# DomhnallBoyle/lip2speech-unit

Hardware: AMD Instinct MI355X
Metric: real-time factor (audio-sec/wall-sec), end-to-end lip->16kHz audio, 4s@25fps clips (higher is better)
Workload: dtype fp16; 1 GPU; e2e lip->units->wav (BASELINE configs[3]: AV-HuBERT large 24L + conformer 12x512 + multi_input HiFi-GAN), 4-s 100-frame 88x88 clips, batch 640 per GPU; clips_per_gpu=640, streams=1, clips_per_launch=640, frames_per_clip=100, hipgraph=True, input=uint8 96x96 frames resident in HBM, crop+normalise on device, enc_layers=24, conf_layers=12, parallelism=clip-parallel dp1

## Files before the change

include/lip2speech_hip.h:

```cpp
#ifndef LIP2SPEECH_HIP_H
#define LIP2SPEECH_HIP_H

#include <stddef.h>
#include <stdint.h>

#ifdef __cplusplus
extern "C" {
#endif

#define L2S_ABI_VERSION 16

enum { L2S_F16 = 0, L2S_BF16 = 1, L2S_F32 = 2 };

enum { L2S_OK = 0, L2S_EINVAL = -1, L2S_ESHAPE = -2, L2S_EALIGN = -3, L2S_EUNSUPPORTED = -4 };

enum {
  L2S_ACT_NONE = 0,
  L2S_ACT_RELU = 1,
  L2S_ACT_GELU = 2,
  L2S_ACT_SWISH = 3,
  L2S_ACT_PRELU = 4,
  L2S_ACT_LRELU = 5,
  L2S_ACT_TANH = 6
};
// ... 141 lines not shown
  float slope;
} l2s_respair_final_desc;
int l2s_respair_final(const l2s_respair_final_desc* d, void* stream);

int l2s_basicblock_fused(const void* x, const void* w1, const float* b1, const float* s1, const void* w2, const float* b2,
                         const float* s2, void* y, int n_images, int H, int W, int C, int dtype, void* stream);
int l2s_basiclayer_fused(const void* x, const void* const* w, const float* const* bias, const float* const* slope, int n_blocks,
                         void* y, int n_images, int H, int W, int C, int dtype, void* stream);
int l2s_basicstage128_tail_fused(const void* x0, const void* t0, const void* wa, const float* ba, const float* sa, const void* w1,
                                 const float* b1, const float* s1, const void* w2, const float* b2, const float* s2, void* y,
                                 int n_images, int H, int W, int dtype, void* stream);

int l2s_conv_post_tanh(const float* x, const float* w, float bias, float* wav, int16_t* pcm, const int32_t* lens,
                       int len_mul, int B, int T, int C, int k, void* stream);

int l2s_resblock_fused(const void* xl, const void* w, const float* bias, float* xs, void* xl_out,
                       const int32_t* lens, int len_mul, int B, int T, int C, int k, int d0, int d1, int d2,
                       int accumulate, float slope, int dtype, void* stream);

int l2s_resstage_fused(const void* xl, const void* const* w, const float* const* bias, const int* ks, const int* dils,
                       int n_blocks, float* xs, void* xl_out, const int32_t* lens, int len_mul, int B, int T, int C,
                       float slope, int xs_final, int dtype, void* stream);

int l2s_preprocess_frames(const uint8_t* frames, void* y, int B, int T, int Hin, int Win, int crop, float mean,
                          float std, int dtype, void* stream);

int l2s_mel_spectrogram(const void* wav, int wav_is_i16, int64_t ldw, const int32_t* n_samples, int B, int S, const float* basis,
                        const float* fb, const int32_t* fb_range, float* mel, int ldm, int T_rows, int n_fft, int hop,
                        int n_mels, float floor_, void* stream);

// ... 61 lines not shown
```

lip2speech_unit_amd/_lib.py:

```python
import ctypes
import os

_HERE = os.path.dirname(os.path.abspath(__file__))
LIB_PATH = os.environ.get("L2S_LIB_PATH") or os.path.join(_HERE, "liblip2speech_hip.so")

F16, BF16, F32 = 0, 1, 2
ACT_NONE, ACT_RELU, ACT_GELU, ACT_SWISH, ACT_PRELU, ACT_LRELU, ACT_TANH = range(7)
F_RES_PRE, F_RES_POST, F_ACCUM, F_DUAL, F_MASK, F_OUT_F32, F_RES_F32 = (1 << i for i in range(7))
MODE_LINEAR, MODE_CONV1D, MODE_CONV2D = 0, 1, 2
ABI_VERSION = 16
SEQ_VARIANT_F32, LN_GENERIC, ATTN_RESIDENT = 2000, 10, 1000

_ERR = {-1: "L2S_EINVAL", -2: "L2S_ESHAPE", -3: "L2S_EALIGN", -4: "L2S_EUNSUPPORTED"}


class L2SError(RuntimeError):
    pass


class GemmDesc(ctypes.Structure):
    _fields_ = [
        ("A", ctypes.c_void_p), ("W", ctypes.c_void_p), ("C", ctypes.c_void_p), ("C2", ctypes.c_void_p),
        ("bias", ctypes.c_void_p), ("slope", ctypes.c_void_p), ("R", ctypes.c_void_p), ("lens", ctypes.c_void_p),
        ("M", ctypes.c_int32), ("N", ctypes.c_int32), ("Cin", ctypes.c_int32), ("ntaps", ctypes.c_int32),
# ... 60 lines not shown
    "l2s_splitk_reduce": ([_vp, _i, _i, _vp, _i, _i, _i, _vp], _i),
    "l2s_splitk_reduce_layernorm": ([_vp, _i, _i, _vp, _i, _vp, _vp, _f, _vp, _i, _i, _i, _i, _vp, _i, _i, _i, _vp], _i),
    "l2s_cast_f32_to_16": ([_vp, _i, _vp, _i, _i, _i, _i, _vp], _i),
    "l2s_cast_16_to_f32": ([_vp, _i, _vp, _i, _i, _i, _i, _vp], _i),
    "l2s_broadcast_rows": ([_vp, _i, _vp, _i, _i, _vp, _i, _i, _i, _i, _i, _i, _vp], _i),
    "l2s_transpose_ct_to_tc": ([_vp, _vp, _i, _i, _vp, _i, _i, _i, _i, _i, _vp], _i),
    "l2s_embedding": ([_vp, _vp, _vp, _i, _vp, _i, _i, _i, _i, _vp], _i),
    "l2s_embedding_tokens": ([_vp, _i, _i, _vp, _i, _vp, _i, _vp, _i, _i, _i, _i, _i, _vp], _i),
    "l2s_rows_f32_to_16_masked": ([_vp, _i, _vp, _i, _i, _vp, _i, _i, _i, _i, _i, _vp], _i),
    "l2s_lens_from_mask": ([_vp, _vp, _i, _i, _vp], _i),
    "l2s_basicblock_fused": ([_vp, _vp, _vp, _vp, _vp, _vp, _vp, _vp, _i, _i, _i, _i, _i, _vp], _i),
    "l2s_basiclayer_fused": ([_vp, _vp, _vp, _vp, _i, _vp, _i, _i, _i, _i, _i, _vp], _i),
    "l2s_basicstage128_tail_fused": ([_vp] * 12 + [_i, _i, _i, _i, _vp], _i),
    "l2s_split_hi_lo": ([_vp, _i, _vp, _vp, _i, _i, _f, _vp, _i, _i, _i, _i, _i, _vp], _i),
    "l2s_conv_post_tanh": ([_vp, _vp, _f, _vp, _vp, _vp, _i, _i, _i, _i, _i, _vp], _i),
    "l2s_resblock_fused": ([_vp, _vp, _vp, _vp, _vp, _vp, _i, _i, _i, _i, _i, _i, _i, _i, _i, _f, _i, _vp], _i),
    "l2s_resstage_fused": ([_vp, _vp, _vp, _vp, _vp, _i, _vp, _vp, _vp, _i, _i, _i, _i, _f, _i, _i, _vp], _i),
    "l2s_respair": ([ctypes.POINTER(RespairDesc), _vp], _i),
    "l2s_respair_variant": ([ctypes.POINTER(RespairDesc)], _i),
    "l2s_respair_final": ([ctypes.POINTER(RespairFinalDesc), _vp], _i),
    "l2s_preprocess_frames": ([_vp, _vp, _i, _i, _i, _i, _i, _f, _f, _i, _vp], _i),
    "l2s_mel_spectrogram": ([_vp, _i, ctypes.c_int64, _vp, _i, _i, _vp, _vp, _vp, _vp, _i, _i, _i, _i, _i, _f, _vp], _i),
    "l2s_stft_mel": ([_vp, _i, ctypes.c_int64, _vp, _i, _i, _vp, _vp, _vp, _vp, _i, _i, _i, _i, _i, _i, _f, _f, _vp], _i),
    "l2s_unit_ce": ([_vp, _i, _vp, _i, _vp, _i, _i, _i, _i, _i, _i, _vp, _vp, _vp, _vp, _vp], _i),
    "l2s_mel_l1_sc": ([_vp, _i, _vp, _i, _vp, _i, _i, _i, _i, _vp, _vp, _vp, _vp, _vp], _i),
    "l2s_ctc_loss_workspace": ([_i, _i, _i], ctypes.c_size_t),
    "l2s_ctc_loss": ([_vp, _i, _vp, _i, _i, _i, _i, _i, _vp, _vp, _vp, _i, _vp, ctypes.c_size_t, _vp, _vp], _i),
    "l2s_wave_stem_workspace": ([_i, _i], ctypes.c_size_t),
    "l2s_wave_stem": ([_vp, _i, ctypes.c_int64, _vp, _i, _i, _vp, _vp, _vp, _f, _vp, _i, _i, _i, _vp, ctypes.c_size_t, _i, _vp], _i),
    "l2s_kmeans_assign": ([_vp, _i, _vp, _vp, _vp, _i, _i, _i, _i, _i, _vp, _vp, _vp], _i),
# ... 51 lines not shown
```

lip2speech_unit_amd/ops.py:

```python
import ctypes
import os
from typing import Optional

import torch

from . import _lib
from ._lib import (ACT_GELU, ACT_LRELU, ACT_NONE, ACT_PRELU, ACT_RELU, ACT_SWISH, ACT_TANH, BF16, F16, F32, F_ACCUM,
                   F_DUAL, F_MASK, F_OUT_F32, F_RES_F32, F_RES_POST, F_RES_PRE, MODE_CONV1D, MODE_CONV2D,
                   MODE_LINEAR, GemmDesc, L2SError, check)

_TORCH16 = {F16: torch.float16, BF16: torch.bfloat16, F32: torch.float32}
_DTYPE_NAME = {F16: "f16", BF16: "bf16", F32: "f32"}


class KernelProfiler:

    def __init__(self, detail=False):
        self.records = []
        self.detail = detail

    def summary(self):
        torch.cuda.synchronize()
        agg = {}
        for key, fl, by, e0, e1, shape in self.records:
# ... 375 lines not shown
    sp = (ctypes.c_void_p * n)(*[_ptr(_req(s_, torch.float32, "slope")) for s_ in slopes])
    M = float(n_images) * H * W
    _run("l2s_basiclayer_fused", lambda: _lib.load().l2s_basiclayer_fused(
        _ptr(x), wp, bp, sp, n // 2, _ptr(y), n_images, H, W, C, dtype, _stream()),
        flops=2.0 * n * M * C * C * 9, nbytes=2 * 2 * M * C)


def split_hi_lo(x, hi, lo, *, B, T, C, act=0, slope=0.0, ldx=None, ld16=None, lens=None, len_mul=1, dtype=F16):
    _run("l2s_split_hi_lo", lambda: _lib.load().l2s_split_hi_lo(_ptr(x), ldx or C, _ptr(hi), _ptr(lo), ld16 or C, act, float(slope),
                                                                _ptr(lens), len_mul, B, T, C, dtype, _stream()))


def conv_post_tanh(x, w, bias, wav, pcm, *, B, T, C, k, lens=None, len_mul=1):
    _run("l2s_conv_post_tanh", lambda: _lib.load().l2s_conv_post_tanh(_ptr(x), _ptr(w), float(bias), _ptr(wav), _ptr(pcm), _ptr(lens), len_mul, B,
                                         T, C, k, _stream()))


def resblock_fused(xl, w, bias, xs, xl_out, *, B, T, C, k, dil, accumulate, slope, lens=None, len_mul=1, dtype=F16):
    _run(f"l2s_resblock_fused<C{C},k{k}>", lambda: _lib.load().l2s_resblock_fused(
        _ptr(xl), _ptr(w), _ptr(bias), _ptr(xs), _ptr(xl_out), _ptr(lens), len_mul, B, T, C, k, dil[0], dil[1], dil[2],
        int(bool(accumulate)), float(slope), dtype, _stream()),
        flops=2.0 * B * T * C * C * k * 6, nbytes=B * T * C * (2 + 4 + (4 if accumulate else 0) + (2 if xl_out is not None else 0)))


def resstage_fused(xl, ws, biases, xs, xl_out, *, B, T, C, ks, dils, slope, lens=None, len_mul=1, dtype=F16, xs_final=True):
    n = len(ws)
    wp = (ctypes.c_void_p * n)(*[_ptr(_req(w, _TORCH16[dtype], "w")) for w in ws])
    bp = (ctypes.c_void_p * n)(*[_ptr(_req(b_, torch.float32, "bias")) for b_ in biases])
    kk = (ctypes.c_int * n)(*[int(k) for k in ks])
    dd = (ctypes.c_int * (3 * n))(*[int(d) for dl in dils for d in dl])
# ... 538 lines not shown
    "embedding_tokens": "(Tensor tok, Tensor table, Tensor(a!) y, *, int B, int L, int C, int token_offset=4, int? ldt=None, "
                        "int? ldy=None, Tensor? lens=None, int len_mul=1, int dtype=0) -> ()",
    "rows_f32_to_16_masked": "(Tensor x, Tensor(a!) y, *, int B, int T, int C, int? ldx=None, int? ldy=None, int col0=0, "
                             "Tensor? lens=None, int len_mul=1, int dtype=0) -> ()",
    "lens_from_mask": "(Tensor? padding_mask, int B, int T, Device device) -> Tensor",
    "basicblock_fused": "(Tensor x, Tensor w1, Tensor b1, Tensor s1, Tensor w2, Tensor b2, Tensor s2, Tensor(a!) y, *, int n_images, "
                        "int H, int W, int C=64, int dtype=0) -> ()",
    "basiclayer_fused": _BL,
    "basicstage128_tail_fused": "(Tensor x0, Tensor t0, Tensor wa, Tensor ba, Tensor sa, Tensor w1, Tensor b1, Tensor s1, Tensor w2, "
                                "Tensor b2, Tensor s2, Tensor(a!) y, *, int n_images, int H, int W, int dtype=0) -> ()",
    "split_hi_lo": "(Tensor x, Tensor(a!) hi, Tensor(b!) lo, *, int B, int T, int C, int act=0, float slope=0.0, int? ldx=None, "
                   "int? ld16=None, Tensor? lens=None, int len_mul=1, int dtype=0) -> ()",
    "conv_post_tanh": _CPT,
    "resblock_fused": "(Tensor xl, Tensor w, Tensor bias, Tensor(a!) xs, Tensor(b!)? xl_out, *, int B, int T, int C, int k, int[] dil, "
                      "bool accumulate, float slope, Tensor? lens=None, int len_mul=1, int dtype=0) -> ()",
    "resstage_fused": "(Tensor xl, Tensor[] ws, Tensor[] biases, Tensor(a!) xs, Tensor(b!)? xl_out, *, int B, int T, int C, int[] ks, "
                      "int[] dils, float slope, Tensor? lens=None, int len_mul=1, int dtype=0, bool xs_final=True) -> ()",
    "respair": _RP,
    "respair_final": "(Tensor[] xs_l, Tensor[] w1s, Tensor[] b1s, Tensor[] w2s, Tensor[] b2s, Tensor(a!) y, *, int B, int T, int C, int[] ks, "
                     "int[] dils, float slope, Tensor? lens=None, int len_mul=1, int dtype=0) -> ()",
    "preprocess_frames": "(Tensor frames, Tensor(a!) y, *, int B, int T, int Hin, int Win, int crop=88, float mean=0.421, "
                         "float std=0.165, int dtype=0) -> ()",
    "mel_spectrogram": "(Tensor wav, Tensor(a!) mel, Tensor basis, Tensor fb, Tensor fb_range, *, int B, int S, int T_rows, "
                       "Tensor? n_samples=None, int? ldw=None, int? ldm=None, int n_fft=640, int hop=160, int n_mels=80, "
                       "float floor=1e-05) -> ()",
    "stft_mel": "(Tensor wav, Tensor(a!) mel, Tensor basis, Tensor fb, Tensor fb_range, *, int B, int S, int T_rows, int n_fft, int hop, "
                "int pad, float mag_eps=0.0, Tensor? n_samples=None, int? ldw=None, int? ldm=None, int n_mels=80, "
                "float floor=1e-05) -> ()",
    "unit_ce": "(Tensor logits, Tensor target, Tensor(a!) nll, Tensor(b!) smooth, Tensor(c!) n_correct, Tensor(d!) n_tok, *, int B, "
               "int T2, int V, int? ldl=None, int? ldt=None, Tensor? lens=None, int len_mul=2, int pad_idx=1, "
# ... 22 lines not shown
                  "int B, int S, int ldf, Tensor? n_samples=None, int? ldx=None, int? ldk=None) -> ()",
    "stoi_scores": "(Tensor bands, Tensor n_kept, Tensor(a!) seg, Tensor(b!) stoi, Tensor(c!) estoi, Tensor(d!) n_segments, *, int B, "
                   "int ldf, int? lds=None) -> ()",
    "wav_gain": "(Tensor wav, Tensor(a!) gain, *, int B, int S, Tensor? n_samples=None, int? ldw=None, float target_dbfs=-30.0) -> ()",
    "stft_mel_power": "(Tensor wav, Tensor(a!) mel, Tensor basis, Tensor fb, Tensor fb_range, *, int B, int S, int T_rows, "
                      "Tensor? n_samples=None, Tensor? n_valid=None, Tensor? scale=None, int? ldw=None, int? ldm=None, int n_fft=400, "
                      "int hop=160, int n_mels=40, int pad=200) -> ()",
    "lstm_layer": "(Tensor xproj, Tensor row_off, Tensor w_hh_p, *, int S, int T, int? n_rows=None, int? ldx=None, int hidden=256, "
                  "Tensor(a!)? h_seq=None, Tensor(b!)? h_last=None) -> ()",
    "spk_embed_head": "(Tensor h_last, Tensor first, Tensor count, Tensor w_t, Tensor bias, Tensor(a!) out, *, int B, "
                      "int? n_rows=None, int hidden=256) -> ()",
}
ENTRY_OF = {n: "l2s_" + n for n in _SCHEMAS}
ENTRY_OF.update({"maxpool2d_3x3s2": "l2s_maxpool2d_3x3s2", "avgpool_hw": "l2s_avgpool_hw"})
HOST_QUERIES = ("l2s_abi_version", "l2s_build_info", "l2s_tapgemm_variant", "l2s_tapgemm_epilogue_family", "l2s_attention_variant", "l2s_layernorm_variant", "l2s_respair_variant",
                "l2s_glu_dwconv_tile", "l2s_beam_decode_workspace",
                "l2s_ctc_beam_workspace", "l2s_ctc_loss_workspace", "l2s_wave_stem_workspace", "l2s_kmeans_nearest_workspace",
                "l2s_kmeans_update_workspace", "l2s_kmeans_pp_workspace")
ALIASES = {"frontend3d_stem": "stem_pool_fused", "resnet_trunk": "basiclayer_fused", "linear_epilogue": "tapgemm",
           "posconv_gelu": "tapgemm", "convtranspose1d": "tapgemm", "mel_head": "tapgemm", "mhsa_padmask": "attention",
           "relpos_mhsa": "attention", "conformer_conv_module": "glu_dwconv_swish", "greedy_unit_decode": "greedy_decode",
           "resblock1": "respair", "tanh_to_int16": "conv_post_tanh"}

_TORCH_LIB = torch.library.Library("lip2speech", "DEF")


def _fake_none(*a, **k):
    return None


def _fake_beam_decode(logits, *, B, T2, V, beam, ldl=None, lens=None, len_mul=1, temperature=1.0, lenpen=1.0):
# ... 58 lines not shown
```

lip2speech_unit_amd/packing.py:

```python
import itertools
from typing import Dict, List

import torch

_clock = itertools.count(1)


def _device(dev):
    dev = torch.device(dev)
    if dev.type == "cuda" and dev.index is None:
        dev = torch.device("cuda", torch.cuda.current_device())
    return dev


def _invalidate_on_load(module, incompatible_keys):
    module.invalidate()


class PackedState:

    def _init_packed(self):
        self._packed, self._packed_dev, self._derived = None, None, {}
        self._epoch = next(_clock)
        self.register_load_state_dict_post_hook(_invalidate_on_load)
# ... 61 lines not shown
        for j in range(p["ntaps"]):
            i = d_max - (p["off"] - j)
            wf[p["r"] * cout:(p["r"] + 1) * cout, i] = wp[:, j]
    if fold == 1:
        return {"w": wf.reshape(stride * cout, S * cin).contiguous(), "ntaps": S, "off": d_max, "n": stride * cout, "fold": 1}
    f, N = fold, stride * cout
    D_max, D_min = (f - 1 + d_max) // f, (d_max - (S - 1)) // f
    S2 = D_max - D_min + 1
    w2 = torch.zeros(f * N, S2, f * cin, dtype=w.dtype)
    for b in range(f):
        for i in range(S):
            m = b + d_max - i
            D, a = m // f, m % f
            w2[b * N:(b + 1) * N, D_max - D, a * cin:(a + 1) * cin] = wf[:, i]
    return {"w": w2.reshape(f * N, S2 * f * cin).contiguous(), "ntaps": S2, "off": D_max, "n": f * N, "fold": f}
```

lip2speech_unit_amd/vocoder.py:

```python
import os

import torch
import torch.nn as nn

from . import ops
from .ops import ACT_GELU, ACT_LRELU, F_ACCUM, F_DUAL, F_MASK, F_RES_POST, MODE_CONV1D
from .packing import PackedState, convtranspose_fused, convtranspose_phases, pack_conv1d

LRELU_SLOPE = 0.1
FUSED_PAIR = os.environ.get("L2S_RESPAIR", "1") != "0"
FUSED_PAIR256 = os.environ.get("L2S_RESPAIR256", "1") != "0"
PAIR_MIN_TILES = int(os.environ.get("L2S_RESPAIR_MIN_TILES", "64"))
PAIR_ROWS = {256: 128, 128: 256, 64: 512}
FUSED_UPS = os.environ.get("L2S_FUSED_UPS", "1") != "0"
FUSED_UPS_MAX_CIN = int(os.environ.get("L2S_FUSED_UPS_MAX_CIN", "128"))
FUSED_STAGE = os.environ.get("L2S_RESSTAGE", "1") != "0"
FUSED_FINAL = os.environ.get("L2S_RESPAIR_FINAL", "1") != "0"
SKIP_DEAD_XS = os.environ.get("L2S_SKIP_DEAD_XS", "1") != "0"


class AttrDict(dict):

    def __init__(self, *args, **kwargs):
        super().__init__(*args, **kwargs)
        self.__dict__ = self


def get_padding(kernel_size, dilation=1):
    return int((kernel_size * dilation - dilation) / 2)

# ... 5 lines not shown
        self.weight_g = nn.Parameter(torch.ones(g_dim0, 1, 1))
        self.weight_v = nn.Parameter(torch.zeros(*shape))
        self.bias = nn.Parameter(torch.zeros(bias_n))

    def effective_weight(self):
        if hasattr(self, "weight") and isinstance(getattr(self, "weight"), torch.Tensor):
            return self.weight.detach().float()
        v, g = self.weight_v.detach().float(), self.weight_g.detach().float()
        return v * (g / v.pow(2).sum(dim=(1, 2), keepdim=True).sqrt())

    def remove_weight_norm(self):
        if "weight_g" in self._parameters:
            w = self.effective_weight()
            del self._parameters["weight_g"], self._parameters["weight_v"]
            self.weight = nn.Parameter(w)


class ResBlock1(nn.Module):
    def __init__(self, h, channels, kernel_size=3, dilation=(1, 3, 5)):
        super().__init__()
        self.channels, self.kernel_size, self.dilation = channels, kernel_size, tuple(dilation)
        self.convs1 = nn.ModuleList([_WN((channels, channels, kernel_size), channels, channels) for _ in dilation])
        self.convs2 = nn.ModuleList([_WN((channels, channels, kernel_size), channels, channels) for _ in dilation])

    def remove_weight_norm(self):
        for m in list(self.convs1) + list(self.convs2):
            m.remove_weight_norm()


class Generator(nn.Module, PackedState):
# ... 25 lines not shown
        for m in self.ups:
            m.remove_weight_norm()
        for m in self.resblocks:
            m.remove_weight_norm()
        self.conv_pre.remove_weight_norm()
        self.conv_post.remove_weight_norm()
        self.invalidate()

    def _conv_pre_weight(self):
        return self.conv_pre.effective_weight()

    def _pack_generator(self, dev):
        t16 = ops.torch_dtype(self.dtype)
        h = self.h
        third = 1.0 / self.num_kernels
        P = {"pre_w": pack_conv1d(self._conv_pre_weight()).to(dev, t16).contiguous(),
             "pre_b": self.conv_pre.bias.detach().float().to(dev).contiguous(), "stages": []}
        for i, (u, k) in enumerate(zip(h.upsample_rates, h.upsample_kernel_sizes)):
            w = self.ups[i].effective_weight()
            if i > 0:
                w = w * third
            st = {"u": u, "cout": w.shape[1], "cin": w.shape[0],
                  "phases": [dict(ph, w=ph["w"].to(dev, t16).contiguous()) for ph in
                             convtranspose_phases(w, u, (k - u) // 2)],
                  "b": self.ups[i].bias.detach().float().to(dev).contiguous(), "rbs": []}
            if FUSED_UPS and w.shape[0] <= FUSED_UPS_MAX_CIN:
                fold = 2 if (w.shape[0] == 32 and u * w.shape[1] == 32) else 1
                f = convtranspose_fused(w, u, (k - u) // 2, fold=fold)
                st["fused"] = dict(f, w=f["w"].to(dev, t16).contiguous(), b=st["b"].repeat(u * fold).contiguous())
            for j in range(self.num_kernels):
                rb = self.resblocks[i * self.num_kernels + j]
                convs = []
                for c1, c2, d in zip(rb.convs1, rb.convs2, rb.dilation):
                    convs.append({
                        "w1": pack_conv1d(c1.effective_weight()).to(dev, t16).contiguous(),
                        "b1": c1.bias.detach().float().to(dev).contiguous(), "d": d,
                        "w2": pack_conv1d(c2.effective_weight()).to(dev, t16).contiguous(),
                        "b2": c2.bias.detach().float().to(dev).contiguous()})
                e = {"k": rb.kernel_size, "convs": convs, "dil": tuple(rb.dilation)}
                C = w.shape[1]
                if C in (16, 32) and rb.kernel_size in (3, 7, 11) and len(rb.dilation) == 3:
                    kpad = ((rb.kernel_size * C + 31) // 32) * 32
                    wf = torch.zeros(6, C, kpad)
                    bf = torch.zeros(6, C)
# ... 82 lines not shown
        P, dt = self._packed["gen"], self.dtype
        t16 = ops.torch_dtype(dt)
        dev = x_l.device
        T, mul = T0, base_mul
        xs = None
        for si, st in enumerate(P["stages"]):
            u, C = st["u"], st["cout"]
            To, M_in = T * u, B * T
            mul *= u
            M = B * To
            pair_stage = FUSED_PAIR and (C in (64, 128) or (C == 256 and FUSED_PAIR256)) and all(
                rb["k"] <= 11 and max(rb["dil"]) * (rb["k"] - 1) // 2 <= (28 if C == 256 else 32) for rb in st["rbs"])
            pair_stage = pair_stage and B * -(-To // PAIR_ROWS[C]) >= PAIR_MIN_TILES
            fused_stage = all("fw" in rb for rb in st["rbs"])
            xl = torch.empty(M, C, device=dev, dtype=t16)
            if (pair_stage or fused_stage) and "fused" in st:
                x, f = None, st["fused"]
                fd = f["fold"] if T % f["fold"] == 0 and (mul // u) % f["fold"] == 0 else 0
                if fd == 0:
                    raise ops.L2SError("folded ConvTranspose needs an even number of input steps per clip")
                ops.tapgemm(x_l, f["w"], xl, M=M_in // fd, N=f["n"], Cin=st["cin"] * fd, ntaps=f["ntaps"], mode=MODE_CONV1D,
                            T_out=T // fd, T_in=T // fd, stride=1, dil=-1, off=f["off"], bias=f["b"], act=ACT_LRELU,
                            act_slope=LRELU_SLOPE, lens=lens, mask_T=T // fd, mask_mul=mul // u // fd, flags=F_MASK, dtype=dt)
            elif pair_stage or fused_stage:
                x = None
                for ph in st["phases"]:
                    ops.tapgemm(x_l, ph["w"], xl, M=M_in, N=C, Cin=st["cin"], ntaps=ph["ntaps"], mode=MODE_CONV1D, T_out=T,
                                T_in=T, stride=1, dil=-1, off=ph["off"], out_row_mul=u, out_row_add=ph["r"], bias=st["b"],
                                act=ACT_LRELU, act_slope=LRELU_SLOPE, lens=lens, mask_T=To, mask_mul=mul, flags=F_MASK,
                                dtype=dt)
            else:
                x = torch.empty(M, C, device=dev, dtype=t16)
                for ph in st["phases"]:
                    ops.tapgemm(x_l, ph["w"], x, M=M_in, N=C, Cin=st["cin"], ntaps=ph["ntaps"], mode=MODE_CONV1D, T_out=T,
                                T_in=T, stride=1, dil=-1, off=ph["off"], out_row_mul=u, out_row_add=ph["r"], bias=st["b"],
                                C2=xl, ldc2=C, lens=lens, mask_T=To, mask_mul=mul, flags=F_DUAL | F_MASK,
                                slope2=LRELU_SLOPE, dtype=dt)
            nxt = torch.empty(M, C, device=dev, dtype=t16)
            last_stage = si == len(P["stages"]) - 1
            final_fused = pair_stage and FUSED_FINAL and SKIP_DEAD_XS and not last_stage and len(st["rbs"]) <= 3
            xs = None if final_fused else torch.empty(M, C, device=dev, dtype=torch.float32)
            if pair_stage:
                finals = []
                for j, rb in enumerate(st["rbs"]):
                    cur_l = xl
# ... 148 lines not shown
        fw = torch.zeros(Etp, Etp)
        fw[:Et, :Et] = fc.weight.detach().float().cpu()
        fb = torch.zeros(Etp)
        fb[:Et] = fc.bias.detach().float().cpu()
        return table, cw, cb, fw, fb

    def pack(self, dev):
        t16 = ops.torch_dtype(self.dtype)
        P = {"gen": self._pack_generator(dev)}
        P["table"] = self.dict.weight.detach().to(dev, t16).contiguous()
        ct = self.layer[0]
        P["up_phases"] = [dict(ph, w=ph["w"].to(dev, t16).contiguous())
                          for ph in convtranspose_phases(ct.weight.detach().float(), 2, 1)]
        P["up_b"] = ct.bias.detach().float().to(dev).contiguous()
        P["fc_w"], P["fc_b"] = self.fc.weight.detach().to(dev, t16).contiguous(), self.fc.bias.detach().float().to(dev).contiguous()
        P["sp_w"], P["sp_b"] = self.spkr.weight.detach().to(dev, t16).contiguous(), self.spkr.bias.detach().float().to(dev).contiguous()
        if self.text_supervision:
            table, cw, cb, fw, fb = self._text_weights()
            P["t_table"] = table.to(dev, t16).contiguous()
            P["t_phases"] = [dict(ph, w=ph["w"].to(dev, t16).contiguous()) for ph in convtranspose_phases(cw, 2, 1)]
            P["t_up_b"], P["t_fc_w"], P["t_fc_b"] = cb.to(dev), fw.to(dev, t16).contiguous(), fb.to(dev)
        self._set_packed(dev, P)

    def _check_text(self, t):
        if self.text_supervision and t is None:
            raise ValueError("this vocoder is text-supervised (models_multi_input.py:75-77): pass the frame labels (t_label)")
        if t is not None and not self.text_supervision:
            raise ValueError("frame labels given to a vocoder without text supervision")

    def forward_rows(self, code, mel, spkr, lens=None, t_label=None):
        dev = code.device
# ... 82 lines not shown
            assert t_rows.dtype == torch.int32 and t_rows.shape[0] == B and t_rows.shape[1] >= L and t_rows.stride(1) == 1
            text = (t_rows, t_rows.stride(0), src_lens, 2)

        def fill(P, cat, emb, Cin, dt):
            ops.embedding_tokens(tokens, P["table"], emb, B=B, L=L, C=self.h.embedding_dim, token_offset=token_offset,
                                 ldt=tokens.stride(0), lens=src_lens, len_mul=2, dtype=dt)
            ops.rows_f32_to_16_masked(mel_rows, cat, B=B, T=2 * L, C=nm, ldy=Cin, col0=0, lens=src_lens, len_mul=4, dtype=dt)
        return self._rows(fill, spkr, src_lens, 2, B, L, dev, text)

    def _rows(self, fill, spkr, lens, lm, B, L, dev, text=None):
        P, dt, h = self.packed(dev), self.dtype, self.h
        t16 = ops.torch_dtype(dt)
        E, nm = h.embedding_dim, self.num_mels
        T0 = 2 * L
        Ct = P["t_table"].shape[1] if self.text_supervision else 0
        Cin = nm + 2 * E + Ct
        cat = torch.empty(B * T0, Cin, device=dev, dtype=t16)
        emb = torch.empty(B * L, E, device=dev, dtype=t16)
        fill(P, cat, emb, Cin, dt)
        up = torch.empty(B * T0, E, device=dev, dtype=t16)
        for ph in P["up_phases"]:
            ops.tapgemm(emb, ph["w"], up, M=B * L, N=E, Cin=E, ntaps=ph["ntaps"], mode=MODE_CONV1D, T_out=L, T_in=L,
                        stride=1, dil=-1, off=ph["off"], out_row_mul=2, out_row_add=ph["r"], bias=P["up_b"],
                        act=ACT_GELU, lens=lens, mask_T=T0, mask_mul=2 * lm, flags=F_MASK, dtype=dt)
        ops.tapgemm(up, P["fc_w"], cat[:, nm:], M=B * T0, N=E, Cin=E, ldc=Cin, bias=P["fc_b"], lens=lens, mask_T=T0,
                    mask_mul=2 * lm, flags=F_MASK, dtype=dt)
        if Ct:
            tok, ldt, tlens, tmul = text
            temb = torch.empty(B * L, Ct, device=dev, dtype=t16)
            ops.embedding_tokens(tok, P["t_table"], temb, B=B, L=L, C=Ct, token_offset=0, ldt=ldt, lens=tlens, len_mul=tmul,
                                 dtype=dt)
            tup = torch.empty(B * T0, Ct, device=dev, dtype=t16)
            for ph in P["t_phases"]:
                ops.tapgemm(temb, ph["w"], tup, M=B * L, N=Ct, Cin=Ct, ntaps=ph["ntaps"], mode=MODE_CONV1D, T_out=L, T_in=L,
                            stride=1, dil=-1, off=ph["off"], out_row_mul=2, out_row_add=ph["r"], bias=P["t_up_b"],
                            act=ACT_GELU, lens=lens, mask_T=T0, mask_mul=2 * lm, flags=F_MASK, dtype=dt)
            ops.tapgemm(tup, P["t_fc_w"], cat[:, nm + E:], M=B * T0, N=Ct, Cin=Ct, ldc=Cin, bias=P["t_fc_b"], lens=lens,
                        mask_T=T0, mask_mul=2 * lm, flags=F_MASK, dtype=dt)
        spkr = spkr.contiguous()
        if spkr.dtype == torch.float32:
            sp16 = torch.empty(B, spkr.shape[1], device=dev, dtype=t16)
            ops.cast_f32_to_16(spkr, sp16, B, spkr.shape[1], dt)
        else:
            sp16 = spkr.to(t16)
        sp = torch.empty(B, E, device=dev, dtype=t16)
        ops.tapgemm(sp16, P["sp_w"], sp, M=B, N=E, Cin=sp16.shape[1], bias=P["sp_b"], dtype=dt)
        ops.broadcast_rows(sp, cat, B=B, T=T0, C=E, ldy=Cin, col0=nm + E + Ct, lens=lens, len_mul=2 * lm, dtype=dt)
        G = P["gen"]
        c0 = G["pre_b"].shape[0]
        x_l = torch.empty(B * T0, c0, device=dev, dtype=t16)
        ops.tapgemm(cat, G["pre_w"], x_l, M=B * T0, N=c0, Cin=Cin, ntaps=7, mode=MODE_CONV1D, T_out=T0, T_in=T0,
                    stride=1, dil=1, off=-3, bias=G["pre_b"], act=ACT_LRELU, act_slope=LRELU_SLOPE, lens=lens,
                    mask_T=T0, mask_mul=2 * lm, flags=F_MASK, dtype=dt)
        return self.generator_rows(x_l, lens, B, T0, 2 * lm)

    def forward(self, **kwargs):
        wav, _ = self.forward_rows(kwargs["code"], kwargs["mel"], kwargs["spkr"], kwargs.get("lens"), t_label=kwargs.get("t_label"))
        return wav.unsqueeze(1)
```

Before: 14080 audio-sec/wall-sec.

## Add dedicated upsample+LReLU kernel with k-step sparsity masks and pad conv_pre Cin

Measured after the change: 14150 audio-sec/wall-sec (median of 6 runs). No clear change (+0.5%).

```diff
diff --git a/include/lip2speech_hip.h b/include/lip2speech_hip.h
--- a/include/lip2speech_hip.h
+++ b/include/lip2speech_hip.h
@@ -179,6 +179,10 @@
 int l2s_conv_post_tanh(const float* x, const float* w, float bias, float* wav, int16_t* pcm, const int32_t* lens,
                        int len_mul, int B, int T, int C, int k, void* stream);
 
+int l2s_upsample_lrelu(const void* x, const void* w, const float* bias, void* y, const int32_t* lens, int len_mul, int B, int T,
+                       int Cin, int N, int ntaps, int off, const uint32_t* kmask, float slope, int dtype, void* stream);
+int l2s_upsample_tile(int Cin, int N);
+
 int l2s_resblock_fused(const void* xl, const void* w, const float* bias, float* xs, void* xl_out,
                        const int32_t* lens, int len_mul, int B, int T, int C, int k, int d0, int d1, int d2,
                        int accumulate, float slope, int dtype, void* stream);
diff --git a/lip2speech_unit_amd/_lib.py b/lip2speech_unit_amd/_lib.py
--- a/lip2speech_unit_amd/_lib.py
+++ b/lip2speech_unit_amd/_lib.py
@@ -98,6 +98,8 @@
     "l2s_basicstage128_tail_fused": ([_vp] * 12 + [_i, _i, _i, _i, _vp], _i),
     "l2s_split_hi_lo": ([_vp, _i, _vp, _vp, _i, _i, _f, _vp, _i, _i, _i, _i, _i, _vp], _i),
     "l2s_conv_post_tanh": ([_vp, _vp, _f, _vp, _vp, _vp, _i, _i, _i, _i, _i, _vp], _i),
+    "l2s_upsample_lrelu": ([_vp, _vp, _vp, _vp, _vp, _i, _i, _i, _i, _i, _i, _i, _vp, _f, _i, _vp], _i),
+    "l2s_upsample_tile": ([_i, _i], _i),
     "l2s_resblock_fused": ([_vp, _vp, _vp, _vp, _vp, _vp, _i, _i, _i, _i, _i, _i, _i, _i, _i, _f, _i, _vp], _i),
     "l2s_resstage_fused": ([_vp, _vp, _vp, _vp, _vp, _i, _vp, _vp, _vp, _i, _i, _i, _i, _f, _i, _i, _vp], _i),
     "l2s_respair": ([ctypes.POINTER(RespairDesc), _vp], _i),
diff --git a/lip2speech_unit_amd/csrc/upsample.hip b/lip2speech_unit_amd/csrc/upsample.hip
--- /dev/null
+++ b/lip2speech_unit_amd/csrc/upsample.hip
@@ -0,0 +1,277 @@
+#include "tapgemm_common.h"
+#include <cstdlib>
+
+using namespace l2s;
+
+namespace {
+
+struct UpsArgs {
+  const uint16_t* X; const uint16_t* W; const float* bias; uint16_t* Y; const int32_t* lens;
+  int len_mul, B, T, tile_rows, tiles_per_clip, ntiles;
+  float slope;
+};
+
+constexpr int UPS_TAPS = 3;
+
+template <int CIN, int N>
+struct UpsCfg {
+  static constexpr int WC = (CIN == 128) ? 4 : 1;
+  static constexpr int WM = 4 / WC;
+  static constexpr int NP = N / 32 / WC;
+  static constexpr int MI = (CIN == 128) ? 8 : 4;
+  static constexpr int TM = WM * MI * 16;
+  static constexpr int PROWS = TM + 8;
+  static constexpr int HALVES = CIN / 64;
+  static constexpr int PLANE_B = PROWS * 128;
+  static constexpr int BUF_B = HALVES * PLANE_B;
+  static constexpr int SMEM = 2 * BUF_B;
+  static constexpr int KS = UPS_TAPS * CIN / 32;
+};
+
+template <typename ET, int CIN, int N, uint64_t MASKS, int NT, unsigned TBS>
+__global__ __launch_bounds__(256, 2) void upsample_lrelu_kernel(const UpsArgs a) {
+  using C = UpsCfg<CIN, N>;
+  constexpr int MI = C::MI, NP = C::NP, KPT = CIN / 32, KS = NT * KPT, K = UPS_TAPS * CIN;
+  static_assert(C::WC == 1 || NP == 1, "a wave's pairs share one tap window");
+  extern __shared__ __attribute__((aligned(16))) uint16_t lds[];
+  const int tid = threadIdx.x, lane = tid & 63;
+  const int wave = __builtin_amdgcn_readfirstlane(tid >> 6);
+  const int lm = lane & 15, lg = lane >> 4;
+  const int srow = lane >> 3, schunk = (lane & 7) ^ (srow & 7);
+  const int wm = wave / C::WC, wc = wave - wm * C::WC;
+  const uint16_t* zero = reinterpret_cast<const uint16_t*>(&g_zero16);
+  const int my_n = (a.ntiles - (int)blockIdx.x + (int)gridDim.x - 1) / (int)gridDim.x;
+  if (my_n <= 0) return;
+  const uint32_t lds_base = (uint32_t)(uintptr_t)(lptr_t)lds;
+
+  auto pair_mask = [](int jp) -> unsigned { return (unsigned)((MASKS >> (12 * jp)) & 0xfffu); };
+  const int tb = (int)((TBS >> (2 * (wc * NP))) & 3u);
+  auto tile_origin = [&](int i, int& b, int& q0) {
+    const int L = blockIdx.x + i * gridDim.x;
+    b = __builtin_amdgcn_readfirstlane(L / a.tiles_per_clip);
+    q0 = (L - b * a.tiles_per_clip) * a.tile_rows;
+  };
+  auto issue_patch = [&](int i, int buf) {
+    int b, q0;
+    tile_origin(i, b, q0);
+    constexpr int NINS = C::HALVES * (C::PROWS / 8);
+    for (int ins = wave; ins < NINS; ins += 4) {
+      const int hp = ins / (C::PROWS / 8), blk = ins - hp * (C::PROWS / 8);
+      const int ts = q0 - 1 + blk * 8 + srow;
+      const uint16_t* g = ((unsigned)ts < (unsigned)a.T) ? a.X + ((int64_t)b * a.T + ts) * CIN + hp * 64 + schunk * 8 : zero;
+      __builtin_amdgcn_global_load_lds((gptr_t)g, (lptr_t)(lds + (buf * C::BUF_B + hp * C::PLANE_B + blk * 1024) / 2), 16, 0, 0);
+    }
+  };
+
+  frag16 wf[NP][2][KS];
+  f32x4_t bj[NP][2];
+#pragma unroll
+  for (int jp = 0; jp < NP; ++jp) {
+    const int J = wc * NP + jp;
+#pragma unroll
+    for (int s2 = 0; s2 < 2; ++s2) {
+      const int n = 32 * J + 8 * (lm >> 2) + 4 * s2 + (lm & 3);
+#pragma unroll
+      for (int s = 0; s < KS; ++s)
+        if ((pair_mask(jp) >> s) & 1u) wf[jp][s2][s].u = *reinterpret_cast<const uint4*>(a.W + (int64_t)n * K + tb * CIN + s * 32 + lg * 8);
+      const float4 q = *reinterpret_cast<const float4*>(a.bias + 32 * J + 8 * lg + 4 * s2);
+      bj[jp][s2] = f32x4_t{q.x, q.y, q.z, q.w};
+    }
+  }
+#pragma unroll
+  for (int jp = 0; jp < NP; ++jp)
+#pragma unroll
+    for (int s2 = 0; s2 < 2; ++s2) {
+#pragma unroll
+      for (int s = 0; s < KS; ++s)
+        if ((pair_mask(jp) >> s) & 1u) asm volatile("" : "+v"(wf[jp][s2][s].h));
+      asm volatile("" : "+v"(bj[jp][s2]));
+    }
+  uint32_t aoff[KS];
+#pragma unroll
+  for (int s = 0; s < KS; ++s) {
+    const int tl = s / KPT, kk = s - tl * KPT, hp = kk >> 1, ks2 = kk & 1;
+    const int pr = wm * MI * 16 + lm + 2 - (tb + tl);
+    aoff[s] = (uint32_t)(hp * C::PLANE_B + pr * 128 + (((ks2 * 4 + lg) ^ (pr & 7)) << 4));
+  }
+  constexpr unsigned ANY = [] {
+    unsigned m = 0;
+    for (int jp = 0; jp < NP; ++jp) m |= (unsigned)((MASKS >> (12 * jp)) & 0xfffu);
+    return m;
+  }();
+
+  issue_patch(0, 0);
+  f32x4_t acc[MI][2 * NP];
+  frag16 fa[2][MI];
+  auto read_a = [&](int s, int slot, uint32_t pb) {
+    const uint32_t ad = pb + aoff[s];
+    lds_read_b128<0>(fa[slot][0], ad); lds_read_b128<2048>(fa[slot][1], ad);
+    lds_read_b128<4096>(fa[slot][2], ad); lds_read_b128<6144>(fa[slot][3], ad);
+    if constexpr (MI == 8) {
+      lds_read_b128<8192>(fa[slot][4], ad); lds_read_b128<10240>(fa[slot][5], ad);
+      lds_read_b128<12288>(fa[slot][6], ad); lds_read_b128<14336>(fa[slot][7], ad);
+    }
+  };
+
+  for (int it = 0; it < my_n; ++it) {
+    wait_vmcnt<0>();
+    __builtin_amdgcn_s_barrier();
+    asm volatile("" ::: "memory");
+    if (it + 1 < my_n) issue_patch(it + 1, (it + 1) & 1);
+    const uint32_t pb = lds_base + (uint32_t)((it & 1) * C::BUF_B);
+#pragma unroll
+    for (int i = 0; i < MI; ++i)
+#pragma unroll
+      for (int j = 0; j < 2 * NP; ++j) acc[i][j] = f32x4_t{0.f, 0.f, 0.f, 0.f};
+
+    constexpr int FIRST = __builtin_ctz(ANY);
+    read_a(FIRST, 0, pb);
+    int slot = 0;
+#pragma unroll
+    for (int s = 0; s < KS; ++s) {
+      if (!((ANY >> s) & 1u)) continue;
+      int nxt = -1;
+#pragma unroll
+      for (int s3 = KS - 1; s3 > s; --s3)
+        if ((ANY >> s3) & 1u) nxt = s3;
+      if (nxt >= 0) {
+        read_a(nxt, slot ^ 1, pb);
+        lds_wait_n<MI>();
+      } else {
+        lds_wait_n<0>();
+      }
+#pragma unroll
+      for (int jp = 0; jp < NP; ++jp) {
+        if ((pair_mask(jp) >> s) & 1u) {
+#pragma unroll
+          for (int i = 0; i < MI; ++i) {
+            acc[i][2 * jp] = ET::mfma(wf[jp][0][s], fa[slot][i], acc[i][2 * jp]);
+            acc[i][2 * jp + 1] = ET::mfma(wf[jp][1][s], fa[slot][i], acc[i][2 * jp + 1]);
+          }
+        }
+      }
+      slot ^= 1;
+    }
+
+    int b, q0;
+    tile_origin(it, b, q0);
+    int valid = a.T;
+    if (a.lens) {
+      int len_b;
+      const int32_t* lp = a.lens + b;
+      asm volatile("s_load_dword %0, %1, 0x0\n\ts_waitcnt lgkmcnt(0)" : "=s"(len_b) : "s"(lp) : "memory");
+      const int v = len_b * a.len_mul;
+      valid = v < a.T ? v : a.T;
+    }
+    const int row_end = (q0 + a.tile_rows < a.T) ? q0 + a.tile_rows : a.T;
+    uint16_t* yrow = a.Y + ((int64_t)b * a.T + q0) * N + wc * NP * 32 + 8 * lg;
+    const float slope = a.slope;
+#pragma unroll
+    for (int i = 0; i < MI; ++i) {
+      const int g0 = q0 + (wm * MI + i) * 16;
+      if (g0 >= row_end) break;
+      const int q = g0 + lm;
+      const bool st = q < row_end;
+      uint16_t* dst = yrow + (int64_t)((wm * MI + i) * 16 + lm) * N;
+      if (g0 >= valid) {
+        if (st) {
+#pragma unroll
+          for (int jp = 0; jp < NP; ++jp) *reinterpret_cast<uint4*>(dst + 32 * jp) = make_uint4(0u, 0u, 0u, 0u);
+        }
+        continue;
+      }
+      const bool partial = g0 + 16 > valid;
+#pragma unroll
+      for (int jp = 0; jp < NP; ++jp) {
+        float v[8];
+#pragma unroll
+        for (int e = 0; e < 8; ++e) {
+          const float x = acc[i][2 * jp + (e >> 2)][e & 3] + bj[jp][e >> 2][e & 3];
+          v[e] = __builtin_amdgcn_fmed3f(x, x * slope, __builtin_inff());
+        }
+        uint4 pk = make_uint4(ET::pack2(v[0], v[1]), ET::pack2(v[2], v[3]), ET::pack2(v[4], v[5]), ET::pack2(v[6], v[7]));
+        if (partial && q >= valid) pk = make_uint4(0u, 0u, 0u, 0u);
+        if (st) *reinterpret_cast<uint4*>(dst + 32 * jp) = pk;
+      }
+    }
+  }
+  wait_vmcnt<0>();
+}
+
+constexpr uint64_t mask4(unsigned m0, unsigned m1, unsigned m2, unsigned m3) {
+  return (uint64_t)m0 | ((uint64_t)m1 << 12) | ((uint64_t)m2 << 24) | ((uint64_t)m3 << 36);
+}
+constexpr uint64_t M64_PHASES = mask4(0x3c, 0x0f, 0, 0);
+constexpr uint64_t M64_FOLD2 = mask4(0x2c, 0x0d, 0, 0);
+constexpr uint64_t M64_DENSE = mask4(0x3f, 0x3f, 0, 0);
+constexpr unsigned TB128_PHASES = 1u | (1u << 2);
+
+bool covers(uint64_t masks, int nt, unsigned tbs, int kpt, int np_wave, const uint32_t* kmask, int npairs) {
+  if (!kmask) return false;
+  for (int J = 0; J < npairs; ++J) {
+    const unsigned local = (unsigned)((masks >> (12 * (J % np_wave))) & 0xfffu) & ((1u << (nt * kpt)) - 1u);
+    const unsigned global = local << (((tbs >> (2 * J)) & 3u) * kpt);
+    if (kmask[J] & ~global) return false;
+  }
+  return true;
+}
+
+int ups_tile_rows(int Cin, int N) {
+  int tm = 0;
+  if (Cin == 64 && N == 64) tm = UpsCfg<64, 64>::TM;
+  if (Cin == 128 && N == 128) tm = UpsCfg<128, 128>::TM;
+  if (!tm) return 0;
+  const char* e = getenv("L2S_UPS_TILE");
+  const int v = e ? atoi(e) : 0;
+  return (v >= 16 && v < tm && v % 16 == 0) ? v : tm;
+}
+
+template <typename ET, int CIN, int N, uint64_t MASKS, int NT, unsigned TBS>
+int launch_ups(UpsArgs a, hipStream_t st) {
+  using C = UpsCfg<CIN, N>;
+  auto kern = upsample_lrelu_kernel<ET, CIN, N, MASKS, NT, TBS>;
+  static L2sSmemOptIn opt_in;
+  if (int e = l2s_smem_opt_in(kern, C::SMEM, opt_in)) return e;
+  constexpr int resident = 512;
+  const char* e = getenv("L2S_UPS_SLOTS");
+  const int sv = e ? atoi(e) : 0;
+  const int slots = sv >= 1 && sv < resident ? sv : resident;
+  const int grid = a.ntiles < slots ? a.ntiles : slots;
+  hipLaunchKernelGGL(kern, dim3(grid), dim3(256), C::SMEM, st, a);
+  L2S_CHECK_LAUNCH();
+  return L2S_OK;
+}
+
+template <typename ET>
+int launch_ups_shape(const UpsArgs& a, int Cin, const uint32_t* kmask, hipStream_t st) {
+  if (Cin == 64) {
+    if (covers(M64_FOLD2, 3, 0, 2, 2, kmask, 2)) return launch_ups<ET, 64, 64, M64_FOLD2, 3, 0>(a, st);
+    if (covers(M64_PHASES, 3, 0, 2, 2, kmask, 2)) return launch_ups<ET, 64, 64, M64_PHASES, 3, 0>(a, st);
+    return launch_ups<ET, 64, 64, M64_DENSE, 3, 0>(a, st);
+  }
+  if (covers(0xff, 2, TB128_PHASES, 4, 1, kmask, 4)) return launch_ups<ET, 128, 128, 0xff, 2, TB128_PHASES>(a, st);
+  return launch_ups<ET, 128, 128, 0xfff, 3, 0>(a, st);
+}
+
+}
+extern "C" int l2s_upsample_tile(int Cin, int N) { return ups_tile_rows(Cin, N); }
+
+extern "C" int l2s_upsample_lrelu(const void* x, const void* w, const float* bias, void* y, const int32_t* lens, int len_mul, int B,
+                                  int T, int Cin, int N, int ntaps, int off, const uint32_t* kmask, float slope, int dtype,
+                                  void* stream) {
+  if (!x || !w || !bias || !y) return L2S_EINVAL;
+  if (B <= 0 || T <= 0 || len_mul <= 0) return L2S_ESHAPE;
+  if (dtype != L2S_F16 && dtype != L2S_BF16) return dtype == L2S_F32 ? L2S_EUNSUPPORTED : L2S_EINVAL;
+  const int tile = ups_tile_rows(Cin, N);
+  if (!tile || ntaps != UPS_TAPS || off != 1 || !(slope > 0.f && slope <= 1.f)) return L2S_EUNSUPPORTED;
+  if ((int64_t)B * T > 0x7fffffff / 2) return L2S_EUNSUPPORTED;
+  if ((((uintptr_t)x | (uintptr_t)w | (uintptr_t)y | (uintptr_t)bias) & 15) != 0) return L2S_EALIGN;
+  UpsArgs a;
+  a.X = (const uint16_t*)x; a.W = (const uint16_t*)w; a.bias = bias; a.Y = (uint16_t*)y; a.lens = lens;
+  a.len_mul = len_mul; a.B = B; a.T = T; a.tile_rows = tile;
+  a.tiles_per_clip = (T + tile - 1) / tile;
+  a.ntiles = B * a.tiles_per_clip;
+  a.slope = slope;
+  hipStream_t st = (hipStream_t)stream;
+  return dtype == L2S_F16 ? launch_ups_shape<ElemF16>(a, Cin, kmask, st) : launch_ups_shape<ElemBF16>(a, Cin, kmask, st);
+}
diff --git a/lip2speech_unit_amd/ops.py b/lip2speech_unit_amd/ops.py
--- a/lip2speech_unit_amd/ops.py
+++ b/lip2speech_unit_amd/ops.py
@@ -413,6 +413,27 @@
 def conv_post_tanh(x, w, bias, wav, pcm, *, B, T, C, k, lens=None, len_mul=1):
     _run("l2s_conv_post_tanh", lambda: _lib.load().l2s_conv_post_tanh(_ptr(x), _ptr(w), float(bias), _ptr(wav), _ptr(pcm), _ptr(lens), len_mul, B,
                                          T, C, k, _stream()))
+
+
+def upsample_tile(Cin, N):
+    return _lib.load().l2s_upsample_tile(int(Cin), int(N))
+
+
+def upsample_lrelu(x, w, bias, y, *, B, T, Cin, N, ntaps, off, slope, kmask=None, lens=None, len_mul=1, dtype=F16):
+    t16 = _TORCH16[dtype]
+    _req(x, t16, "x"), _req(w, t16, "w"), _req(y, t16, "y"), _req(bias, torch.float32, "bias")
+    if lens is not None and lens.dtype != torch.int32:
+        raise L2SError("lens must be int32")
+    if _extent(x) < B * T * Cin or _extent(y) < B * T * N or w.numel() < N * ntaps * Cin or bias.numel() < N:
+        raise L2SError("upsample_lrelu: operand smaller than its shape")
+    km = None
+    if kmask is not None:
+        if len(kmask) != N // 32:
+            raise L2SError("kmask: one word per 32 output channels")
+        km = (ctypes.c_uint32 * len(kmask))(*[int(m) for m in kmask])
+    _run(f"l2s_upsample_lrelu<C{Cin}>", lambda: _lib.load().l2s_upsample_lrelu(
+        _ptr(x), _ptr(w), _ptr(bias), _ptr(y), _ptr(lens), len_mul, B, T, Cin, N, ntaps, off, km, float(slope), dtype, _stream()),
+        flops=2.0 * B * T * N * ntaps * Cin, nbytes=2.0 * B * T * (Cin + N) + 2.0 * N * ntaps * Cin, shape=f"M{B * T} N{N} K{ntaps * Cin}")
 
 
 def resblock_fused(xl, w, bias, xs, xl_out, *, B, T, C, k, dil, accumulate, slope, lens=None, len_mul=1, dtype=F16):
@@ -981,6 +1002,8 @@
     "conv_post_tanh": _CPT,
     "resblock_fused": "(Tensor xl, Tensor w, Tensor bias, Tensor(a!) xs, Tensor(b!)? xl_out, *, int B, int T, int C, int k, int[] dil, "
                       "bool accumulate, float slope, Tensor? lens=None, int len_mul=1, int dtype=0) -> ()",
+    "upsample_lrelu": "(Tensor x, Tensor w, Tensor bias, Tensor(a!) y, *, int B, int T, int Cin, int N, int ntaps, int off, float slope, "
+                      "int[]? kmask=None, Tensor? lens=None, int len_mul=1, int dtype=0) -> ()",
     "resstage_fused": "(Tensor xl, Tensor[] ws, Tensor[] biases, Tensor(a!) xs, Tensor(b!)? xl_out, *, int B, int T, int C, int[] ks, "
                       "int[] dils, float slope, Tensor? lens=None, int len_mul=1, int dtype=0, bool xs_final=True) -> ()",
     "respair": _RP,
@@ -1033,7 +1056,7 @@
 ENTRY_OF = {n: "l2s_" + n for n in _SCHEMAS}
 ENTRY_OF.update({"maxpool2d_3x3s2": "l2s_maxpool2d_3x3s2", "avgpool_hw": "l2s_avgpool_hw"})
 HOST_QUERIES = ("l2s_abi_version", "l2s_build_info", "l2s_tapgemm_variant", "l2s_tapgemm_epilogue_family", "l2s_attention_variant", "l2s_layernorm_variant", "l2s_respair_variant",
-                "l2s_glu_dwconv_tile", "l2s_beam_decode_workspace",
+                "l2s_upsample_tile", "l2s_glu_dwconv_tile", "l2s_beam_decode_workspace",
                 "l2s_ctc_beam_workspace", "l2s_ctc_loss_workspace", "l2s_wave_stem_workspace", "l2s_kmeans_nearest_workspace",
                 "l2s_kmeans_update_workspace", "l2s_kmeans_pp_workspace")
 ALIASES = {"frontend3d_stem": "stem_pool_fused", "resnet_trunk": "basiclayer_fused", "linear_epilogue": "tapgemm",
diff --git a/lip2speech_unit_amd/packing.py b/lip2speech_unit_amd/packing.py
--- a/lip2speech_unit_amd/packing.py
+++ b/lip2speech_unit_amd/packing.py
@@ -99,3 +99,16 @@
             D, a = m // f, m % f
             w2[b * N:(b + 1) * N, D_max - D, a * cin:(a + 1) * cin] = wf[:, i]
     return {"w": w2.reshape(f * N, S2 * f * cin).contiguous(), "ntaps": S2, "off": D_max, "n": f * N, "fold": f}
+
+
+def kstep_mask(w: torch.Tensor) -> List[int]:
+    n, k = w.shape
+    nz = (w.reshape(n // 32, 32, k // 32, 32) != 0).any(dim=3).any(dim=1)
+    return [sum(1 << s for s in range(k // 32) if bool(nz[j, s])) for j in range(n // 32)]
+
+
+def pad_conv1d_cin(w: torch.Tensor, cin_to: int) -> torch.Tensor:
+    cout, cin, k = w.shape
+    if cin_to == cin:
+        return w
+    return torch.cat([w, w.new_zeros(cout, cin_to - cin, k)], 1)
diff --git a/lip2speech_unit_amd/vocoder.py b/lip2speech_unit_amd/vocoder.py
--- a/lip2speech_unit_amd/vocoder.py
+++ b/lip2speech_unit_amd/vocoder.py
@@ -5,7 +5,7 @@
 
 from . import ops
 from .ops import ACT_GELU, ACT_LRELU, F_ACCUM, F_DUAL, F_MASK, F_RES_POST, MODE_CONV1D
-from .packing import PackedState, convtranspose_fused, convtranspose_phases, pack_conv1d
+from .packing import PackedState, convtranspose_fused, convtranspose_phases, kstep_mask, pack_conv1d, pad_conv1d_cin
 
 LRELU_SLOPE = 0.1
 FUSED_PAIR = os.environ.get("L2S_RESPAIR", "1") != "0"
@@ -14,6 +14,9 @@
 PAIR_ROWS = {256: 128, 128: 256, 64: 512}
 FUSED_UPS = os.environ.get("L2S_FUSED_UPS", "1") != "0"
 FUSED_UPS_MAX_CIN = int(os.environ.get("L2S_FUSED_UPS_MAX_CIN", "128"))
+UPS_STREAM = os.environ.get("L2S_UPS_STREAM", "1") != "0"
+UPS_STREAM_MIN_ROWS = int(os.environ.get("L2S_UPS_STREAM_MIN_ROWS", str(64 * 1024)))
+PRE_PAD = os.environ.get("L2S_PRE_PAD", "1") != "0"
 FUSED_STAGE = os.environ.get("L2S_RESSTAGE", "1") != "0"
 FUSED_FINAL = os.environ.get("L2S_RESPAIR_FINAL", "1") != "0"
 SKIP_DEAD_XS = os.environ.get("L2S_SKIP_DEAD_XS", "1") != "0"
@@ -49,6 +52,39 @@
             w = self.effective_weight()
             del self._parameters["weight_g"], self._parameters["weight_v"]
             self.weight = nn.Parameter(w)
+
+
+def pack_upsample(w, bias, u, k, dev, dtype):
+    t16 = ops.torch_dtype(dtype)
+    st = {"u": u, "cout": w.shape[1], "cin": w.shape[0],
+          "phases": [dict(ph, w=ph["w"].to(dev, t16).contiguous()) for ph in convtranspose_phases(w, u, (k - u) // 2)],
+          "b": bias.to(dev).contiguous()}
+    if FUSED_UPS and w.shape[0] <= FUSED_UPS_MAX_CIN:
+        fold = 2 if (w.shape[0] == 32 and u * w.shape[1] == 32) else 1
+        f = convtranspose_fused(w, u, (k - u) // 2, fold=fold)
+        st["fused"] = dict(f, w=f["w"].to(dev, t16).contiguous(), b=st["b"].repeat(u * fold).contiguous())
+        if dtype in (ops.F16, ops.BF16) and f["ntaps"] == 3 and f["off"] == 1 and ops.upsample_tile(w.shape[0] * fold, f["n"]) > 0:
+            st["fused"]["kmask"] = kstep_mask(f["w"].to(t16).float())
+    return st
+
+
+def upsample_xl(st, x_l, xl, lens, B, T, mul, dt):
+    u, C, M_in = st["u"], st["cout"], B * T
+    f = st.get("fused")
+    if f is not None and T % f["fold"] == 0 and (mul // u) % f["fold"] == 0:
+        fd = f["fold"]
+        if UPS_STREAM and "kmask" in f and M_in // fd >= UPS_STREAM_MIN_ROWS:
+            ops.upsample_lrelu(x_l, f["w"], f["b"], xl, B=B, T=T // fd, Cin=st["cin"] * fd, N=f["n"], ntaps=f["ntaps"], off=f["off"],
+                               slope=LRELU_SLOPE, kmask=f["kmask"], lens=lens, len_mul=mul // u // fd, dtype=dt)
+        else:
+            ops.tapgemm(x_l, f["w"], xl, M=M_in // fd, N=f["n"], Cin=st["cin"] * fd, ntaps=f["ntaps"], mode=MODE_CONV1D,
+                        T_out=T // fd, T_in=T // fd, stride=1, dil=-1, off=f["off"], bias=f["b"], act=ACT_LRELU,
+                        act_slope=LRELU_SLOPE, lens=lens, mask_T=T // fd, mask_mul=mul // u // fd, flags=F_MASK, dtype=dt)
+        return
+    for ph in st["phases"]:
+        ops.tapgemm(x_l, ph["w"], xl, M=M_in, N=C, Cin=st["cin"], ntaps=ph["ntaps"], mode=MODE_CONV1D, T_out=T, T_in=T, stride=1,
+                    dil=-1, off=ph["off"], out_row_mul=u, out_row_add=ph["r"], bias=st["b"], act=ACT_LRELU,
+                    act_slope=LRELU_SLOPE, lens=lens, mask_T=T * u, mask_mul=mul, flags=F_MASK, dtype=dt)
 
 
 class ResBlock1(nn.Module):
@@ -104,20 +140,16 @@
         t16 = ops.torch_dtype(self.dtype)
         h = self.h
         third = 1.0 / self.num_kernels
-        P = {"pre_w": pack_conv1d(self._conv_pre_weight()).to(dev, t16).contiguous(),
+        wpre = self._conv_pre_weight()
+        pre_cin = -(-wpre.shape[1] // 64) * 64 if PRE_PAD else wpre.shape[1]
+        P = {"pre_w": pack_conv1d(pad_conv1d_cin(wpre, pre_cin)).to(dev, t16).contiguous(), "pre_cin": pre_cin,
              "pre_b": self.conv_pre.bias.detach().float().to(dev).contiguous(), "stages": []}
         for i, (u, k) in enumerate(zip(h.upsample_rates, h.upsample_kernel_sizes)):
             w = self.ups[i].effective_weight()
             if i > 0:
                 w = w * third
-            st = {"u": u, "cout": w.shape[1], "cin": w.shape[0],
-                  "phases": [dict(ph, w=ph["w"].to(dev, t16).contiguous()) for ph in
-                             convtranspose_phases(w, u, (k - u) // 2)],
-                  "b": self.ups[i].bias.detach().float().to(dev).contiguous(), "rbs": []}
-            if FUSED_UPS and w.shape[0] <= FUSED_UPS_MAX_CIN:
-                fold = 2 if (w.shape[0] == 32 and u * w.shape[1] == 32) else 1
-                f = convtranspose_fused(w, u, (k - u) // 2, fold=fold)
-                st["fused"] = dict(f, w=f["w"].to(dev, t16).contiguous(), b=st["b"].repeat(u * fold).contiguous())
+            st = pack_upsample(w, self.ups[i].bias.detach().float(), u, k, dev, self.dtype)
+            st["rbs"] = []
             for j in range(self.num_kernels):
                 rb = self.resblocks[i * self.num_kernels + j]
                 convs = []
@@ -230,21 +262,9 @@
             pair_stage = pair_stage and B * -(-To // PAIR_ROWS[C]) >= PAIR_MIN_TILES
             fused_stage = all("fw" in rb for rb in st["rbs"])
             xl = torch.empty(M, C, device=dev, dtype=t16)
-            if (pair_stage or fused_stage) and "fused" in st:
-                x, f = None, st["fused"]
-                fd = f["fold"] if T % f["fold"] == 0 and (mul // u) % f["fold"] == 0 else 0
-                if fd == 0:
-                    raise ops.L2SError("folded ConvTranspose needs an even number of input steps per clip")
-                ops.tapgemm(x_l, f["w"], xl, M=M_in // fd, N=f["n"], Cin=st["cin"] * fd, ntaps=f["ntaps"], mode=MODE_CONV1D,
-                            T_out=T // fd, T_in=T // fd, stride=1, dil=-1, off=f["off"], bias=f["b"], act=ACT_LRELU,
-                            act_slope=LRELU_SLOPE, lens=lens, mask_T=T // fd, mask_mul=mul // u // fd, flags=F_MASK, dtype=dt)
-            elif pair_stage or fused_stage:
+            if pair_stage or fused_stage:
                 x = None
-                for ph in st["phases"]:
-                    ops.tapgemm(x_l, ph["w"], xl, M=M_in, N=C, Cin=st["cin"], ntaps=ph["ntaps"], mode=MODE_CONV1D, T_out=T,
-                                T_in=T, stride=1, dil=-1, off=ph["off"], out_row_mul=u, out_row_add=ph["r"], bias=st["b"],
-                                act=ACT_LRELU, act_slope=LRELU_SLOPE, lens=lens, mask_T=To, mask_mul=mul, flags=F_MASK,
-                                dtype=dt)
+                upsample_xl(st, x_l, xl, lens, B, T, mul, dt)
             else:
                 x = torch.empty(M, C, device=dev, dtype=t16)
                 for ph in st["phases"]:
@@ -423,7 +443,11 @@
                           for ph in convtranspose_phases(ct.weight.detach().float(), 2, 1)]
         P["up_b"] = ct.bias.detach().float().to(dev).contiguous()
         P["fc_w"], P["fc_b"] = self.fc.weight.detach().to(dev, t16).contiguous(), self.fc.bias.detach().float().to(dev).contiguous()
-        P["sp_w"], P["sp_b"] = self.spkr.weight.detach().to(dev, t16).contiguous(), self.spkr.bias.detach().float().to(dev).contiguous()
+        sw, sb = self.spkr.weight.detach().float(), self.spkr.bias.detach().float()
+        pad = P["gen"]["pre_cin"] - self._conv_pre_weight().shape[1]
+        if pad:
+            sw, sb = torch.cat([sw, sw.new_zeros(pad, sw.shape[1])], 0), torch.cat([sb, sb.new_zeros(pad)], 0)
+        P["sp_w"], P["sp_b"] = sw.to(dev, t16).contiguous(), sb.to(dev).contiguous()
         if self.text_supervision:
             table, cw, cb, fw, fb = self._text_weights()
             P["t_table"] = table.to(dev, t16).contiguous()
@@ -536,7 +560,8 @@
         E, nm = h.embedding_dim, self.num_mels
         T0 = 2 * L
         Ct = P["t_table"].shape[1] if self.text_supervision else 0
-        Cin = nm + 2 * E + Ct
+        Cin = P["gen"]["pre_cin"]
+        Es = Cin - (nm + E + Ct)
         cat = torch.empty(B * T0, Cin, device=dev, dtype=t16)
         emb = torch.empty(B * L, E, device=dev, dtype=t16)
         fill(P, cat, emb, Cin, dt)
@@ -565,9 +590,9 @@
             ops.cast_f32_to_16(spkr, sp16, B, spkr.shape[1], dt)
         else:
             sp16 = spkr.to(t16)
-        sp = torch.empty(B, E, device=dev, dtype=t16)
-        ops.tapgemm(sp16, P["sp_w"], sp, M=B, N=E, Cin=sp16.shape[1], bias=P["sp_b"], dtype=dt)
-        ops.broadcast_rows(sp, cat, B=B, T=T0, C=E, ldy=Cin, col0=nm + E + Ct, lens=lens, len_mul=2 * lm, dtype=dt)
+        sp = torch.empty(B, Es, device=dev, dtype=t16)
+        ops.tapgemm(sp16, P["sp_w"], sp, M=B, N=Es, Cin=sp16.shape[1], bias=P["sp_b"], dtype=dt)
+        ops.broadcast_rows(sp, cat, B=B, T=T0, C=Es, ldy=Cin, col0=nm + E + Ct, lens=lens, len_mul=2 * lm, dtype=dt)
         G = P["gen"]
         c0 = G["pre_b"].shape[0]
         x_l = torch.empty(B * T0, c0, device=dev, dtype=t16)
```
